# WQCG/blitzdg

Measured on AMD Instinct MI355X. Metric: element-DOF updates/sec (sw2d RHS + LSERK4 stage, N=4, 1M tris), higher is better.
Workload: dtype f64

## Files before the change

blitzdg_amd/csrc/hip/sw2d_affine_kernel.hpp:

```cpp
#pragma once
#include "sw2d_kernels.hpp"

namespace bdg_dev {

template <int N>
struct AffineOps {
    using E = Elem<N>;
    static constexpr int OFF_D = 0;
    static constexpr int OFF_LIFT = 2 * E::Np * E::Np;
    static constexpr int DOUBLES = OFF_LIFT + E::NFN * E::Np;
};

__device__ __forceinline__ double fast_rcp(double x) {
    double r = __builtin_amdgcn_rcp(x);
    r = fma(fma(-x, r, 1.0), r, r);
    r = fma(fma(-x, r, 1.0), r, r);
    return r;
}

__device__ __forceinline__ double fast_sqrt(double x) {
    x = fmax(x, 1e-290);
    const double y = __builtin_amdgcn_rsq(x);
    double g = x * y, h = 0.5 * y;
    const double r = fma(-h, g, 0.5);
    g = fma(g, r, g);
    h = fma(h, r, h);
    g = fma(fma(-g, g, x), h, g);
    return g;
}

template <typename T>
__device__ __forceinline__ T ld_row(const T* row, unsigned byteOff) {
    return *reinterpret_cast<const T*>(reinterpret_cast<const char*>(row) + byteOff);
}
template <typename T>
__device__ __forceinline__ void st_row(T* row, unsigned byteOff, T v) {
    *reinterpret_cast<T*>(reinterpret_cast<char*>(row) + byteOff) = v;
}

struct PhysParams {
    const double* sx;
    const double* sy;
    const double* fcor;
    const double* fmat;
    double fconst, cd, slope, dragSign;
    const double* H;
    const int* obc;
    const double* lam;
    const double* spongeField;
    double tide;
};

template <int N>
__device__ __forceinline__ unsigned link_node(unsigned code, int n) {
    using E = Elem<N>;
    const bool rev = (code & 4u) != 0;
    const unsigned f = code & 3u;
    const unsigned m0 = rev ? E::fmask(0, N - n) : E::fmask(0, n);
    const unsigned m1 = rev ? E::fmask(1, N - n) : E::fmask(1, n);
    const unsigned m2 = rev ? E::fmask(2, N - n) : E::fmask(2, n);
    return f == 0u ? m0 : (f == 1u ? m1 : m2);
}

constexpr int STAGE_VMAP = -1;

template <int N, int MODE, int PHYS = 0, bool TRACER = false, bool SPONGE = false, int KIND = STAGE_VMAP>
__global__ __launch_bounds__(256) void sw2d_stage_affine_kernel(const StageParams p, const PhysParams ph) {
    using E = Elem<N>;
    constexpr int Np = E::Np, Nfp = E::Nfp, NFN = E::NFN;
    constexpr bool kLinks = KIND != STAGE_VMAP;
    static_assert(!kLinks || (MODE == MODE_LSERK && PHYS == 0 && !TRACER && !SPONGE), "face links: three-field LSERK stages");
    constexpr bool kReadRes = MODE == MODE_LSERK && KIND != STAGE_FIRST;
    constexpr bool kWriteRes = KIND != STAGE_LAST;

    const unsigned nwg = gridDim.x, xcd = blockIdx.x % 8u, q8 = nwg / 8u, r8 = nwg % 8u;
    const unsigned tile = (xcd < r8 ? xcd * (q8 + 1u) : r8 * (q8 + 1u) + (xcd - r8) * q8) + blockIdx.x / 8u;
    const unsigned k = static_cast<unsigned>(p.kbegin) + tile * blockDim.x + threadIdx.x;
    if (k >= static_cast<unsigned>(p.kend)) return;
    const unsigned k8 = k * 8u, k4 = k * 4u;

    const long long ld = p.ld, plane = static_cast<long long>(Np) * ld;
    const double* __restrict__ ops = p.opsAffine;
    const double* __restrict__ qin = p.qin;

    int idx[kLinks ? 1 : NFN];
    unsigned lnk[kLinks ? 3 : 1];
    if constexpr (kLinks) {
        const unsigned* __restrict__ fl = reinterpret_cast<const unsigned*>(p.faceLink);
#pragma unroll
        for (int f = 0; f < 3; ++f) lnk[f] = ld_row(fl + f * ld, k4);
    } else {
#pragma unroll
        for (int j = 0; j < NFN; ++j) idx[j] = ld_row(p.vmapP + j * ld, k4);
    }
    double h[Np], hu[Np], hv[Np], hN[TRACER ? Np : 1];
#pragma unroll
    for (int n = 0; n < Np; ++n) {
        h[n] = ld_row(qin + n * ld, k8);
        hu[n] = ld_row(qin + plane + n * ld, k8);
        hv[n] = ld_row(qin + 2 * plane + n * ld, k8);
        if constexpr (TRACER) hN[n] = ld_row(qin + 3 * plane + n * ld, k8);
    }
    const double* __restrict__ ag = p.ageo;
    const double rx = ld_row(ag, k8), sx = ld_row(ag + ld, k8), ry = ld_row(ag + 2 * ld, k8), sy = ld_row(ag + 3 * ld, k8);
    double fnx[3], fny[3], fsc[3];
#pragma unroll
    for (int f = 0; f < 3; ++f) {
        fnx[f] = ld_row(ag + (4 + f) * ld, k8);
        fny[f] = ld_row(ag + (7 + f) * ld, k8);
        fsc[f] = ld_row(ag + (10 + f) * ld, k8);
    }
    double ssx[PHYS != 0 ? Np : 1], ssy[PHYS != 0 ? Np : 1], sfc[PHYS != 0 ? Np : 1];
    if constexpr (PHYS != 0) {
#pragma unroll
        for (int i = 0; i < Np; ++i) { ssx[i] = 0.0; ssy[i] = 0.0; sfc[i] = ph.fconst; }
        if (ph.sx) {
#pragma unroll
            for (int i = 0; i < Np; ++i) ssx[i] = ld_row(ph.sx + i * ld, k8);
        }
        if (ph.sy) {
#pragma unroll
            for (int i = 0; i < Np; ++i) ssy[i] = ld_row(ph.sy + i * ld, k8);
        }
        if (ph.fcor) {
#pragma unroll
            for (int i = 0; i < Np; ++i) sfc[i] = ld_row(ph.fcor + i * ld, k8);
        }
    }
    __builtin_amdgcn_sched_barrier(0);
    double hP[NFN], huP[NFN], hvP[NFN], hNP[TRACER ? NFN : 1];
    auto gatherFace = [&](int f) {
#pragma unroll
        for (int n = 0; n < Nfp; ++n) {
            const int j = f * Nfp + n;
            const unsigned o8 = static_cast<unsigned>(idx[j] < 0 ? -(idx[j] + 1) : idx[j]) * 8u;
            hP[j] = ld_row(qin, o8);
            huP[j] = ld_row(qin + plane, o8);
            hvP[j] = ld_row(qin + 2 * plane, o8);
            if constexpr (TRACER) hNP[j] = ld_row(qin + 3 * plane, o8);
        }
    };
    constexpr bool kLateFace = TRACER && MODE != MODE_LSERK;
    if constexpr (kLateFace) {
        gatherFace(0);
        gatherFace(1);
    } else if constexpr (kLinks) {
        const unsigned uld = static_cast<unsigned>(ld);
#pragma unroll
        for (int j = 0; j < NFN; ++j) {
            const int f = j / Nfp, n = j % Nfp;
            const unsigned code = lnk[f] >> FaceLink::FACE_SHIFT & 7u;
            const unsigned o8 = (link_node<N>(code, n) * uld + (lnk[f] & FaceLink::SLOT_MASK)) * 8u;
            hP[j] = ld_row(qin, o8);
            huP[j] = ld_row(qin + plane, o8);
            hvP[j] = ld_row(qin + 2 * plane, o8);
        }
    } else {
#pragma unroll
        for (int j = 0; j < NFN; ++j) {
            const unsigned o8 = static_cast<unsigned>(idx[j] < 0 ? -(idx[j] + 1) : idx[j]) * 8u;
            hP[j] = ld_row(qin, o8);
            huP[j] = ld_row(qin + plane, o8);
            hvP[j] = ld_row(qin + 2 * plane, o8);
            if constexpr (TRACER) hNP[j] = ld_row(qin + 3 * plane, o8);
        }
    }
    __builtin_amdgcn_sched_barrier(0);

    const double g = p.g, halfg = 0.5 * p.g;
    double R1[Np], R2[Np], R3[Np], R4[TRACER ? Np : 1];
#pragma unroll
    for (int i = 0; i < Np; ++i) R1[i] = R2[i] = R3[i] = 0.0;
    if constexpr (TRACER) {
#pragma unroll
        for (int i = 0; i < Np; ++i) R4[i] = 0.0;
    }
    if constexpr (PHYS != 0) {
#pragma unroll
        for (int m = 0; m < Np; ++m) {
            const double r = fast_rcp(h[m]);
            const double u = hu[m] * r, v = hv[m] * r;
            const double cdn = ph.cd * fast_sqrt(u * u + v * v);
            const double gh = ph.slope * g * h[m];
            R2[m] = fma(gh, ssx[m], fma(sfc[m], hv[m], -(cdn * u)));
            R3[m] = fma(gh, ssy[m], fma(ph.dragSign * cdn, v, -(sfc[m] * hu[m])));
        }
    }

#pragma unroll
    for (int f = 0; f < 3; ++f) {
        const double nxf = fnx[f], nyf = fny[f];
        double lam = 0.0;
        double uM[Nfp], vM[Nfp], uP[Nfp], vP[Nfp], hq[Nfp], huq[Nfp], hvq[Nfp];
#pragma unroll
        for (int n = 0; n < Nfp; ++n) {
            const int j = f * Nfp + n, m = E::fmask(f, n);
            const double rM = fast_rcp(h[m]);
            uM[n] = hu[m] * rM;
            vM[n] = hv[m] * rM;
            const double spdM = fast_sqrt(uM[n] * uM[n] + vM[n] * vM[n]) + fast_sqrt(g * h[m]);
            hq[n] = hP[j];
            huq[n] = huP[j];
            hvq[n] = hvP[j];
            bool wall;
            if constexpr (kLinks) wall = (lnk[f] & FaceLink::WALL) != 0u;
            else wall = idx[j] < 0;
            if (wall) {
                const double un = hu[m] * nxf + hv[m] * nyf;
                huq[n] = hu[m] - 2 * nxf * un;
                hvq[n] = hv[m] - 2 * nyf * un;
            }
            const double r = fast_rcp(hq[n]);
            uP[n] = huq[n] * r;
            vP[n] = hvq[n] * r;
            const double spdP = fast_sqrt(uP[n] * uP[n] + vP[n] * vP[n]) + fast_sqrt(g * hq[n]);
            lam = fmax(lam, fmax(spdM, spdP));
        }
        const double half_fs = 0.5 * fsc[f];
#pragma unroll
        for (int n = 0; n < Nfp; ++n) {
            const int j = f * Nfp + n, m = E::fmask(f, n);
            const double prM = halfg * h[m] * h[m], prP = halfg * hq[n] * hq[n];
            const double F2M = hu[m] * uM[n] + prM, G2M = hu[m] * vM[n], G3M = hv[m] * vM[n] + prM;
            const double F2P = huq[n] * uP[n] + prP, G2P = huq[n] * vP[n], G3P = hvq[n] * vP[n] + prP;
            const double dh = h[m] - hq[n], dhu = hu[m] - huq[n], dhv = hv[m] - hvq[n];
            const double s1 = half_fs * (dhu * nxf + dhv * nyf - lam * dh);
            const double s2 = half_fs * ((F2M - F2P) * nxf + (G2M - G2P) * nyf - lam * dhu);
            const double s3 = half_fs * ((G2M - G2P) * nxf + (G3M - G3P) * nyf - lam * dhv);
            double s4 = 0.0;
            if constexpr (TRACER)
                s4 = half_fs * ((hN[m] * uM[n] - hNP[j] * uP[n]) * nxf + (hN[m] * vM[n] - hNP[j] * vP[n]) * nyf -
                                lam * (hN[m] - hNP[j]));
#pragma unroll
            for (int i = 0; i < Np; ++i) {
                const double lj = ops[AffineOps<N>::OFF_LIFT + j * Np + i];
                R1[i] = fma(lj, s1, R1[i]);
                R2[i] = fma(lj, s2, R2[i]);
                R3[i] = fma(lj, s3, R3[i]);
                if constexpr (TRACER) R4[i] = fma(lj, s4, R4[i]);
            }
        }
        if constexpr (kLateFace) {
            if (f == 0) {
                gatherFace(2);
                __builtin_amdgcn_sched_barrier(0);
            }
        }
    }

    double old1[Np], old2[Np], old3[Np], old4[TRACER ? Np : 1];
    if constexpr (kReadRes) {
        const double* __restrict__ rs = p.res;
#pragma unroll
        for (int i = 0; i < Np; ++i) {
            old1[i] = ld_row(rs + i * ld, k8);
            old2[i] = ld_row(rs + plane + i * ld, k8);
            old3[i] = ld_row(rs + 2 * plane + i * ld, k8);
            if constexpr (TRACER) old4[i] = ld_row(rs + 3 * plane + i * ld, k8);
        }
    } else if constexpr (MODE == MODE_COMBINE) {
        const double* __restrict__ qb = p.qbase;
#pragma unroll
        for (int i = 0; i < Np; ++i) {
            old1[i] = ld_row(qb + i * ld, k8);
            old2[i] = ld_row(qb + plane + i * ld, k8);
            old3[i] = ld_row(qb + 2 * plane + i * ld, k8);
        }
    }
    __builtin_amdgcn_sched_barrier(0);

#pragma unroll
    for (int m = 0; m < Np; ++m) {
        const double r = fast_rcp(h[m] * p.one);
        const double u = hu[m] * r, v = hv[m] * r;
        const double pr = halfg * h[m] * h[m];
        const double F2 = hu[m] * u + pr, G2 = hu[m] * v, G3 = hv[m] * v + pr;
        const double a1 = -(rx * hu[m] + ry * hv[m]), b1 = -(sx * hu[m] + sy * hv[m]);
        const double a2 = -(rx * F2 + ry * G2), b2 = -(sx * F2 + sy * G2);
        const double a3 = -(rx * G2 + ry * G3), b3 = -(sx * G2 + sy * G3);
        double a4 = 0.0, b4 = 0.0;
        if constexpr (TRACER) {
            const double F4 = hN[m] * u, G4 = hN[m] * v;
            a4 = -(rx * F4 + ry * G4);
            b4 = -(sx * F4 + sy * G4);
        }
#pragma unroll
        for (int i = 0; i < Np; ++i) {
            const double dr = ops[AffineOps<N>::OFF_D + 2 * (m * Np + i)];
            R1[i] = fma(dr, a1, R1[i]);
            R2[i] = fma(dr, a2, R2[i]);
            R3[i] = fma(dr, a3, R3[i]);
            if constexpr (TRACER) R4[i] = fma(dr, a4, R4[i]);
        }
#pragma unroll
        for (int i = 0; i < Np; ++i) {
            const double ds = ops[AffineOps<N>::OFF_D + 2 * (m * Np + i) + 1];
            R1[i] = fma(ds, b1, R1[i]);
            R2[i] = fma(ds, b2, R2[i]);
            R3[i] = fma(ds, b3, R3[i]);
            if constexpr (TRACER) R4[i] = fma(ds, b4, R4[i]);
        }
    }

    if constexpr (PHYS == 2) {
        auto applyFilter = [&](double (&R)[Np]) {
            double T[Np];
#pragma unroll
            for (int i = 0; i < Np; ++i) T[i] = 0.0;
#pragma unroll
            for (int m = 0; m < Np; ++m)
#pragma unroll
                for (int i = 0; i < Np; ++i) T[i] = fma(ph.fmat[m * Np + i], R[m], T[i]);
#pragma unroll
            for (int i = 0; i < Np; ++i) R[i] = T[i];
        };
        applyFilter(R1);
        applyFilter(R2);
        applyFilter(R3);
        if constexpr (TRACER) applyFilter(R4);
    }

    if constexpr (TRACER && MODE == MODE_COMBINE) {
        const double* __restrict__ o4 = p.qbase + 3 * plane;
#pragma unroll
        for (int i = 0; i < Np; ++i) old4[i] = ld_row(o4 + i * ld, k8);
        __builtin_amdgcn_sched_barrier(0);
    }
    if constexpr (MODE == MODE_RHS) {
        double* __restrict__ o = p.rhs;
#pragma unroll
        for (int i = 0; i < Np; ++i) {
            st_row(o + i * ld, k8, R1[i]);
            st_row(o + plane + i * ld, k8, R2[i]);
            st_row(o + 2 * plane + i * ld, k8, R3[i]);
            if constexpr (TRACER) st_row(o + 3 * plane + i * ld, k8, R4[i]);
        }
    } else if constexpr (MODE == MODE_LSERK) {
        double* __restrict__ rs = p.res;
        double* __restrict__ o = p.qout;
        const double a = p.ca, b = p.cb, dt = p.cc;
#pragma unroll
        for (int i = 0; i < Np; ++i) {
            double n1, n2, n3;
            if constexpr (!kLinks) {
                n1 = a * old1[i] + dt * R1[i];
                n2 = a * old2[i] + dt * R2[i];
                n3 = a * old3[i] + dt * R3[i];
            } else if constexpr (kReadRes) {
                n1 = fma(dt, R1[i], a * old1[i]);
                n2 = fma(dt, R2[i], a * old2[i]);
                n3 = fma(dt, R3[i], a * old3[i]);
            } else {
                n1 = dt * R1[i];
                n2 = dt * R2[i];
                n3 = dt * R3[i];
            }
            if constexpr (kWriteRes) {
                st_row(rs + i * ld, k8, n1);
                st_row(rs + plane + i * ld, k8, n2);
                st_row(rs + 2 * plane + i * ld, k8, n3);
            }
            st_row(o + i * ld, k8, h[i] + b * n1);
            st_row(o + plane + i * ld, k8, hu[i] + b * n2);
            st_row(o + 2 * plane + i * ld, k8, hv[i] + b * n3);
            if constexpr (TRACER) {
                const double n4 = a * old4[i] + dt * R4[i];
                st_row(rs + 3 * plane + i * ld, k8, n4);
                st_row(o + 3 * plane + i * ld, k8, hN[i] + b * n4);
            }
        }
    } else {
        static_assert(!SPONGE || MODE == MODE_COMBINE, "the sponge follows a combine step");
        double* __restrict__ o = p.qout;
        const double a = p.ca, b = p.cb, c = p.cc;
        const double sg = p.sponge;
#pragma unroll
        for (int i = 0; i < Np; ++i) {
            const double v2 = a * old2[i] + b * hu[i] + c * R2[i], v3 = a * old3[i] + b * hv[i] + c * R3[i];
            st_row(o + i * ld, k8, a * old1[i] + b * h[i] + c * R1[i]);
            st_row(o + plane + i * ld, k8, SPONGE ? v2 / (1.0 + sg * v2 * v2) : v2);
            st_row(o + 2 * plane + i * ld, k8, SPONGE ? v3 / (1.0 + sg * v3 * v3) : v3);
        }
        if constexpr (TRACER) {
#pragma unroll
            for (int i = 0; i < Np; ++i) st_row(o + 3 * plane + i * ld, k8, a * old4[i] + b * hN[i] + c * R4[i]);
        }
    }
}

}

namespace bdg_dev {

template <int N, int MODE, int WAVES>
__global__ __launch_bounds__(256, WAVES) void sw2d_stage_affine_stream_kernel(const StageParams p) {
    using E = Elem<N>;
    constexpr int Np = E::Np, Nfp = E::Nfp;

    const unsigned nwg = gridDim.x, xcd = blockIdx.x % 8u, q8 = nwg / 8u, r8 = nwg % 8u;
    const unsigned tile = (xcd < r8 ? xcd * (q8 + 1u) : r8 * (q8 + 1u) + (xcd - r8) * q8) + blockIdx.x / 8u;
    const unsigned k = static_cast<unsigned>(p.kbegin) + tile * blockDim.x + threadIdx.x;
    if (k >= static_cast<unsigned>(p.kend)) return;
    const unsigned k8 = k * 8u, k4 = k * 4u;

    const long long ld = p.ld, plane = static_cast<long long>(Np) * ld;
    const double* __restrict__ ops = p.opsAffine;
    const double* __restrict__ qin = p.qin;
    const double* __restrict__ ag = p.ageo;
    const double g = p.g, halfg = 0.5 * p.g;

    double R1[Np], R2[Np], R3[Np];
#pragma unroll
    for (int i = 0; i < Np; ++i) R1[i] = R2[i] = R3[i] = 0.0;

    {
        const double rx = ld_row(ag, k8), sx = ld_row(ag + ld, k8), ry = ld_row(ag + 2 * ld, k8),
                     sy = ld_row(ag + 3 * ld, k8);
        constexpr int VCH = 5, NCH = (Np + VCH - 1) / VCH;
        double hc[2][VCH], huc[2][VCH], hvc[2][VCH];
#pragma unroll
        for (int t = 0; t < VCH; ++t)
            if (t < Np) {
                hc[0][t] = ld_row(qin + t * ld, k8);
                huc[0][t] = ld_row(qin + plane + t * ld, k8);
                hvc[0][t] = ld_row(qin + 2 * plane + t * ld, k8);
            }
#pragma unroll
        for (int c = 0; c < NCH; ++c) {
            const int cur = c & 1, nxt = cur ^ 1;
#pragma unroll
            for (int t = 0; t < VCH; ++t) {
                const int m = (c + 1) * VCH + t;
                if (m < Np) {
                    hc[nxt][t] = ld_row(qin + m * ld, k8);
                    huc[nxt][t] = ld_row(qin + plane + m * ld, k8);
                    hvc[nxt][t] = ld_row(qin + 2 * plane + m * ld, k8);
                }
            }
            __builtin_amdgcn_sched_barrier(0);
#pragma unroll
            for (int t = 0; t < VCH; ++t) {
                const int m = c * VCH + t;
                if (m < Np) {
                    const double h = hc[cur][t], hu = huc[cur][t], hv = hvc[cur][t];
                    const double r = fast_rcp(h);
                    const double u = hu * r, v = hv * r;
                    const double pr = halfg * h * h;
                    const double F2 = hu * u + pr, G2 = hu * v, G3 = hv * v + pr;
                    const double a1 = -(rx * hu + ry * hv), b1 = -(sx * hu + sy * hv);
                    const double a2 = -(rx * F2 + ry * G2), b2 = -(sx * F2 + sy * G2);
                    const double a3 = -(rx * G2 + ry * G3), b3 = -(sx * G2 + sy * G3);
#pragma unroll
                    for (int i = 0; i < Np; ++i) {
                        const double dr = ops[AffineOps<N>::OFF_D + 2 * (m * Np + i)];
                        R1[i] = fma(dr, a1, R1[i]);
                        R2[i] = fma(dr, a2, R2[i]);
                        R3[i] = fma(dr, a3, R3[i]);
                    }
#pragma unroll
                    for (int i = 0; i < Np; ++i) {
                        const double ds = ops[AffineOps<N>::OFF_D + 2 * (m * Np + i) + 1];
                        R1[i] = fma(ds, b1, R1[i]);
                        R2[i] = fma(ds, b2, R2[i]);
                        R3[i] = fma(ds, b3, R3[i]);
                    }
                }
            }
            __builtin_amdgcn_sched_barrier(0);
        }
    }
    __builtin_amdgcn_sched_barrier(0);

#pragma unroll
    for (int f = 0; f < 3; ++f) {
        const double nxf = ld_row(ag + (4 + f) * ld, k8), nyf = ld_row(ag + (7 + f) * ld, k8);
        const double half_fs = 0.5 * ld_row(ag + (10 + f) * ld, k8);
        int idx[Nfp];
        double hM[Nfp], huM[Nfp], hvM[Nfp], hq[Nfp], huq[Nfp], hvq[Nfp];
#pragma unroll
        for (int n = 0; n < Nfp; ++n) idx[n] = ld_row(p.vmapP + (f * Nfp + n) * ld, k4);
#pragma unroll
        for (int n = 0; n < Nfp; ++n) {
            const int m = E::fmask(f, n);
            hM[n] = ld_row(qin + m * ld, k8);
            huM[n] = ld_row(qin + plane + m * ld, k8);
            hvM[n] = ld_row(qin + 2 * plane + m * ld, k8);
        }
#pragma unroll
        for (int n = 0; n < Nfp; ++n) {
            const unsigned o8 = static_cast<unsigned>(idx[n] < 0 ? -(idx[n] + 1) : idx[n]) * 8u;
            hq[n] = ld_row(qin, o8);
            huq[n] = ld_row(qin + plane, o8);
            hvq[n] = ld_row(qin + 2 * plane, o8);
        }
        __builtin_amdgcn_sched_barrier(0);
        double lam = 0.0;
#pragma unroll
        for (int n = 0; n < Nfp; ++n) {
            if (idx[n] < 0) {
                const double un = huM[n] * nxf + hvM[n] * nyf;
                huq[n] = huM[n] - 2 * nxf * un;
                hvq[n] = hvM[n] - 2 * nyf * un;
            }
            const double rM = fast_rcp(hM[n]), rP = fast_rcp(hq[n]);
            const double uM = huM[n] * rM, vM = hvM[n] * rM, uP = huq[n] * rP, vP = hvq[n] * rP;
            const double spdM = fast_sqrt(uM * uM + vM * vM) + fast_sqrt(g * hM[n]);
            const double spdP = fast_sqrt(uP * uP + vP * vP) + fast_sqrt(g * hq[n]);
            lam = fmax(lam, fmax(spdM, spdP));
        }
#pragma unroll
        for (int n = 0; n < Nfp; ++n) {
            const int j = f * Nfp + n;
            const double rM = fast_rcp(hM[n] * p.one), rP = fast_rcp(hq[n] * p.one);
            const double uM = huM[n] * rM, vM = hvM[n] * rM, uP = huq[n] * rP, vP = hvq[n] * rP;
            const double prM = halfg * hM[n] * hM[n], prP = halfg * hq[n] * hq[n];
            const double F2M = huM[n] * uM + prM, G2M = huM[n] * vM, G3M = hvM[n] * vM + prM;
            const double F2P = huq[n] * uP + prP, G2P = huq[n] * vP, G3P = hvq[n] * vP + prP;
            const double dh = hM[n] - hq[n], dhu = huM[n] - huq[n], dhv = hvM[n] - hvq[n];
            const double s1 = half_fs * (dhu * nxf + dhv * nyf - lam * dh);
            const double s2 = half_fs * ((F2M - F2P) * nxf + (G2M - G2P) * nyf - lam * dhu);
            const double s3 = half_fs * ((G2M - G2P) * nxf + (G3M - G3P) * nyf - lam * dhv);
#pragma unroll
            for (int i = 0; i < Np; ++i) {
                const double lj = ops[AffineOps<N>::OFF_LIFT + j * Np + i];
                R1[i] = fma(lj, s1, R1[i]);
                R2[i] = fma(lj, s2, R2[i]);
                R3[i] = fma(lj, s3, R3[i]);
// ... 230 lines not shown
```

blitzdg_amd/csrc/hip/sw2d_device.hip:

```cpp
#include "../host/capi_internal.hpp"
#include "../host/element_order.hpp"
#include "../host/parallel_for.hpp"
#include "blitzdg/LSERK4.hpp"
#include "run_records.hpp"
#include "sw2d_launch.hpp"
#include "sw2d_launch_host.hpp"
#include "sw2d_drifter_kernel.hpp"
#include <algorithm>
#include <atomic>
#include <cmath>
#include <cstdlib>
#include <cstring>
#include <limits>
#include <queue>
#include <stdexcept>
#include <string>
#include <vector>

namespace bdg_dev {

const KernelTable* kernel_table_order1();
const KernelTable* kernel_table_order2();
const KernelTable* kernel_table_order3();
const KernelTable* kernel_table_order4();
// ... 686 lines not shown
                    img[o + 2] = F ? F[i * Np + m] : (i == m ? 1.0 : 0.0);
                }
            for (int j = 0; j < NFN; ++j)
                for (int i = 0; i < Np; ++i)
                    img[static_cast<size_t>(3) * Np * Np + static_cast<size_t>(j) * Np + i] = Lift[i * NFN + j];
            return img;
        };
        opsVd.upload(image(hostDr.data(), hostDs.data(), nullptr, hostLift.data()), bytes, "source ops upload");
        if (!hostFilter.empty())
            opsVdFiltered.upload(image(hostFDr.data(), hostFDs.data(), hostFilter.data(), hostFLift.data()), bytes,
                                 "filtered source ops upload");
    }

    void buildMfma2SourceOps() {
        if (opsMfma2Src.p) return;
        const int MT = kt->mfmaMT, KV = kt->mfmaKV, KF = kt->mfma2KF;
        auto image = [&](const double* Dr, const double* Ds, const double* Lift, const double* F) {
            const size_t tilesD = static_cast<size_t>(MT) * KV * 64, offF = static_cast<size_t>(kt->mfma2OpsDoubles);
            std::vector<double> img(offF + tilesD, 0.0);
            for (int r = 0; r < MT; ++r)
                for (int l = 0; l < 64; ++l) {
                    const int i = 16 * r + (l & 15);
                    if (i >= Np) continue;
                    for (int t = 0; t < KV; ++t) {
                        const int k = 4 * t + (l >> 4);
                        if (k >= Np) continue;
                        const size_t at = (static_cast<size_t>(r) * KV + t) * 64 + l;
                        img[at] = Dr[i * Np + k];
                        img[tilesD + at] = Ds[i * Np + k];
                        img[offF + at] = F ? F[i * Np + k] : (i == k ? 1.0 : 0.0);
                    }
                    for (int f = 0; f < 3; ++f)
                        for (int tf = 0; tf < KF; ++tf) {
                            const int n = 4 * tf + (l >> 4);
                            if (n < Nfp)
                                img[2 * tilesD + ((static_cast<size_t>(r) * 3 + f) * KF + tf) * 64 + l] = Lift[i * NFN + f * Nfp + n];
                        }
                }
            return img;
        };
        opsMfma2Src.upload(image(hostDr.data(), hostDs.data(), hostLift.data(), nullptr), bytes, "mfma2 source ops upload");
        if (!hostFilter.empty())
            opsMfma2SrcFiltered.upload(image(hostFDr.data(), hostFDs.data(), hostFLift.data(), hostFilter.data()), bytes,
                                       "filtered mfma2 source ops upload");
    }
    void buildFilterT() {
        if (filterT.p || hostFilter.empty()) return;
        std::vector<double> ft(static_cast<size_t>(Np) * Np);
        for (int m = 0; m < Np; ++m)
            for (int i = 0; i < Np; ++i) ft[static_cast<size_t>(m) * Np + i] = hostFilter[static_cast<size_t>(i) * Np + m];
        filterT.upload(ft, bytes, "filter upload");
    }

    void monitorReserve(long long steps, const char* fn) const { mon.reserve(steps, fn, "bdg_sw2d"); }
    void drifterReserve(long long steps, const char* fn) const { drf.reserve(steps, fn, "bdg_sw2d"); }
    long long lserkSteps(long long stages) const { return bdg_records::lserkSteps(stageCount, stages, blitzdg::LSERK4::numStages); }
    void monitorLaunch(double* rec, int capacity, int slot) {
        const double* Hm = mon.H.p ? mon.H.p : (hasH ? Hbuf.p : nullptr);
        mon.launch({qcur, Hm, ld, Np, nf, numOwned, g, timeNow}, rec, capacity, slot, bdg_dev::sw2d_monitor_finish_kernel,
                   "sw2d_monitor_finish_kernel launch", bdg_dev::MonRowGauges{mon.row.p}, stream);
    }
    void monitorSample() { monitorLaunch(mon.rec.p, mon.capacity, mon.count++); }
    void drifterLaunch(int mode, double dt, int slot) {
        drf.launch(bdg_dev::sw2d_drifter_kernel, "sw2d_drifter_kernel launch",
                   bdg_dev::TriDriftTables{drf.vert.p, drf.neigh.p, drf.vinvT.p, drf.jac.p}, qcur, ld, N, mode, dt, slot, stream);
    }
    void drifterAdvance(double dt, bool record = true) { drifterLaunch(bdg_dev::kDriftAdvance, dt, drf.takeSlot(record)); }
    void drifterResample() {
        if (drf.on) drifterLaunch(bdg_dev::kDriftSample, 0.0, -1);
    }
    void stepDone(double dt) {
        if (mon.on && ++mon.steps % mon.stride == 0) monitorSample();
        if (drf.on) {
            drf.t = timeNow;
            drifterAdvance(dt);
        }
    }
    void lserkStagesMonitored(int numStages) {
        for (int i = 0; i < numStages; ++i) {
            launchLserkStage();
            if (stageCount % blitzdg::LSERK4::numStages == 0) stepDone(dtStage);
        }
    }
    void lserkStagesExchangedMonitored(double dt, int numStages) {
        if (!mon.on) {
            launchLserkStagesExchanged(dt, numStages);
            return;
        }
        int left = numStages;
        while (left > 0) {
            const int toStep = blitzdg::LSERK4::numStages - static_cast<int>(stageCount % blitzdg::LSERK4::numStages);
            const long long stepsToDue = mon.stride - mon.steps % mon.stride;
            const long long want = toStep + (stepsToDue - 1) * blitzdg::LSERK4::numStages;
            const int piece = static_cast<int>(std::min<long long>(left, want));
            const long long done = lserkSteps(piece);
            launchLserkStagesExchanged(dt, piece);
            left -= piece;
            if (done > 0) {
                mon.steps += done - 1;
                stepDone(dt);
            }
        }
    }

    void reduceDt(double out[2]) {
        const int nblocks = (numOwned + 255) / 256;
        hipCheck(kt->dt(qcur, fscaleNodal, hasH ? Hbuf.p : nullptr, ld, numOwned, g, partials.p,
                        stream), "sw2d_dt_kernel");
        hipLaunchKernelGGL(bdg_dev::sw2d_reduce_kernel, dim3(1), dim3(256), 0, stream, partials.p, nblocks, red2.p);
        hipCheck(hipGetLastError(), "sw2d_reduce_kernel");
        hipCheck(hipMemcpyAsync(out, red2.p, 2 * sizeof(double), hipMemcpyDeviceToHost, stream), "D2H copy");
        hipCheck(hipStreamSynchronize(stream), "reduce sync");
    }
};

namespace {

bool geometryIsAffine(const bdg_sw2d_desc& d, int Np, int Nfp, int K) {
    const double tol = 1e-8;
    std::atomic<bool> ok{true};
    blitzdg::detail::parallelFor(K, [&](int k) {
        const double scale = std::fabs(d.rx[k]) + std::fabs(d.sx[k]) + std::fabs(d.ry[k]) + std::fabs(d.sy[k]);
        for (int n = 1; n < Np; ++n) {
            const size_t o = static_cast<size_t>(n) * K + k;
            if (std::fabs(d.rx[o] - d.rx[k]) > tol * scale || std::fabs(d.sx[o] - d.sx[k]) > tol * scale ||
                std::fabs(d.ry[o] - d.ry[k]) > tol * scale || std::fabs(d.sy[o] - d.sy[k]) > tol * scale)
                ok = false;
        }
        for (int f = 0; f < 3; ++f) {
            const size_t o0 = static_cast<size_t>(f) * Nfp * K + k;
            for (int n = 1; n < Nfp; ++n) {
                const size_t o = o0 + static_cast<size_t>(n) * K;
                if (std::fabs(d.nx[o] - d.nx[o0]) > tol || std::fabs(d.ny[o] - d.ny[o0]) > tol ||
                    std::fabs(d.Fscale[o] - d.Fscale[o0]) > tol * std::fabs(d.Fscale[o0]))
                    ok = false;
            }
        }
    });
    return ok;
}

std::vector<double> matmulHost(const double* A, const double* B, int n, int c) {
    std::vector<double> C(static_cast<size_t>(n) * c, 0.0);
    for (int i = 0; i < n; ++i)
        for (int j = 0; j < c; ++j) {
            double s = 0.0;
            for (int k = 0; k < n; ++k) s += A[i * n + k] * B[k * c + j];
            C[static_cast<size_t>(i) * c + j] = s;
        }
    return C;
}

std::vector<double> affineOpsImage(const double* Dr, const double* Ds, const double* Lift, int Np, int NFN) {
    std::vector<double> img(static_cast<size_t>(2) * Np * Np + static_cast<size_t>(NFN) * Np);
    for (int m = 0; m < Np; ++m)
        for (int i = 0; i < Np; ++i) {
            img[2 * (static_cast<size_t>(m) * Np + i)] = Dr[i * Np + m];
            img[2 * (static_cast<size_t>(m) * Np + i) + 1] = Ds[i * Np + m];
        }
    for (int j = 0; j < NFN; ++j)
        for (int i = 0; i < Np; ++i) img[static_cast<size_t>(2) * Np * Np + static_cast<size_t>(j) * Np + i] = Lift[i * NFN + j];
    return img;
}

bdg_sw2d* createSolver(const bdg_sw2d_desc& d) {
    if (d.order < 1 || d.order > BDG_SW2D_MAX_ORDER)
        throw arg_error("bdg_sw2d_create: order must be 1.." + std::to_string(BDG_SW2D_MAX_ORDER) +
                        " for the register-resident kernels");
    if (d.num_elements < 1) throw arg_error("bdg_sw2d_create: num_elements must be >= 1");
    if (!d.Dr || !d.Ds || !d.Lift || !d.rx || !d.sx || !d.ry || !d.sy || !d.nx || !d.ny || !d.Fscale || !d.vmapP)
        throw arg_error("bdg_sw2d_create: a required table pointer is NULL");
    if (d.num_wall < 0 || (d.num_wall > 0 && !d.mapW)) throw arg_error("bdg_sw2d_create: bad wall-node list");

    const bdg_dev::KernelTable* kt = bdg_dev::kernel_table(d.order);
    if (!kt) throw arg_error("bdg_sw2d_create: no kernels compiled for this order");

    int ndev = 0;
    if (hipGetDeviceCount(&ndev) != hipSuccess || ndev < 1)
        throw hip_error("bdg_sw2d_create: no HIP device available (the sw2d path has no CPU fallback)");
    if (d.device < 0 || d.device >= ndev) throw arg_error("bdg_sw2d_create: device ordinal out of range");

    auto s = std::unique_ptr<bdg_sw2d>(new bdg_sw2d());
    s->kt = kt;
    s->N = d.order; s->Np = kt->Np; s->Nfp = kt->Nfp; s->NFN = 3 * kt->Nfp; s->K = d.num_elements;
    s->device = d.device;
    s->g = d.g;
    if (d.num_fields != 0 && d.num_fields != 3 && d.num_fields != 4)
        throw arg_error("bdg_sw2d_create: num_fields must be 3 or 4");
    s->nf = d.num_fields == 4 ? 4 : 3;
    s->variantD = s->nf == 4 || d.sources != 0;
    s->ld = (static_cast<long long>(s->K) + 63) / 64 * 64;
    s->numInterior = s->numOwned = s->K;
    const int Np = s->Np, Nfp = s->Nfp, NFN = s->NFN, K = s->K;
    const long long ld = s->ld;
    if (static_cast<long long>(Np) * ld * 8 > 4294967295LL)
        throw arg_error("bdg_sw2d_create: Np*K exceeds 2^29 nodes (32-bit byte offsets within a field): partition the "
                        "mesh over more devices");

    const size_t nFaceNodes = static_cast<size_t>(NFN) * K;
    if (d.vmapM)
        for (int k = 0; k < K; ++k)
            for (int f = 0; f < 3; ++f)
                for (int n = 0; n < Nfp; ++n)
                    if (d.vmapM[(static_cast<size_t>(k) * 3 + f) * Nfp + n] != kt->fmask(f, n) + Np * k)
                        throw arg_error("bdg_sw2d_create: vmapM does not follow the warp&blend face-node ordering "
                                        "(Fmask) these kernels are specialised for");
    const long long totalNodes = static_cast<long long>(Np) * K;
    for (size_t i = 0; i < nFaceNodes; ++i)
        if (d.vmapP[i] < 0 || d.vmapP[i] >= totalNodes) throw arg_error("bdg_sw2d_create: vmapP entry out of range");
    for (int i = 0; i < d.num_wall; ++i)
        if (d.mapW[i] < 0 || static_cast<size_t>(d.mapW[i]) >= nFaceNodes)
            throw arg_error("bdg_sw2d_create: wall-node index out of range");

    namespace eo = blitzdg::element_order;
    const bool reorder = (d.flags & BDG_SW2D_REORDER) != 0 ||
                         (!(d.flags & BDG_SW2D_KEEP_ORDER) && eo::renumberingWanted(d.vmapP, K, Np, Nfp, d.order));
    if (reorder) s->permHost = eo::renumbering(d.vmapP, K, Np, Nfp, eo::patchSetting());
    s->affine = !(d.flags & BDG_SW2D_NODAL_GEOMETRY) && geometryIsAffine(d, Np, Nfp, K);
    s->nodalMfma = !s->affine && !(env::nodalVector() && kt->ldsDoubles != 0);

    s->use();
    hipCheck(hipStreamCreateWithFlags(&s->stream, hipStreamNonBlocking), "hipStreamCreate");

    const size_t plane3 = static_cast<size_t>(s->nf) * s->planeSize();
    s->qA.alloc(plane3, s->bytes);
    s->qB.alloc(plane3, s->bytes);
    s->res.alloc(plane3, s->bytes);
    s->aux.alloc(plane3, s->bytes);
    const size_t fplane = static_cast<size_t>(NFN) * ld;
    if (!s->affine) {
        s->geo.alloc(4 * s->planeSize(), s->bytes);
        s->fgeo.alloc(3 * fplane, s->bytes);
        s->ops.alloc(kt->ldsDoubles, s->bytes);
    } else {
        s->fgeo.alloc(fplane, s->bytes);
    }
    s->fscaleNodal = s->affine ? s->fgeo.p : s->fgeo.p + 2 * fplane;
    s->vmapP.alloc(static_cast<size_t>(NFN) * ld, s->bytes);
    s->stage.alloc(static_cast<size_t>(std::max(Np, NFN)) * K, s->bytes);
    s->istage.alloc(static_cast<size_t>(NFN) * K, s->bytes);
    s->partials.alloc(2 * static_cast<size_t>((K + 255) / 256), s->bytes);
    s->red2.alloc(2, s->bytes);
    if (!s->permHost.empty()) s->perm.upload(s->permHost, s->bytes, "perm upload");
    for (auto* b : {&s->qA, &s->qB, &s->res, &s->aux, &s->geo, &s->fgeo})
        if (b->p) hipCheck(hipMemsetAsync(b->p, 0, b->n * sizeof(double), s->stream), "hipMemset");
    hipCheck(hipMemsetAsync(s->vmapP.p, 0, s->vmapP.n * sizeof(int), s->stream), "hipMemset");
    s->qcur = s->qA.p;
    s->qalt = s->qB.p;

    s->hasFilter = d.Filter != nullptr;
    if (!s->affine && kt->ldsDoubles > 0) {
        std::vector<double> img(kt->ldsDoubles, 0.0);
        for (int i = 0; i < Np * Np; ++i) {
            img[2 * i] = d.Dr[i];
            img[2 * i + 1] = d.Ds[i];
        }
        std::copy(d.Lift, d.Lift + static_cast<size_t>(Np) * NFN, img.begin() + 2 * Np * Np);
        if (d.Filter) std::copy(d.Filter, d.Filter + static_cast<size_t>(Np) * Np, img.begin() + 2 * Np * Np + Np * NFN);
        hipCheck(hipMemcpyAsync(s->ops.p, img.data(), img.size() * sizeof(double), hipMemcpyHostToDevice, s->stream),
                 "ops upload");
        hipCheck(hipStreamSynchronize(s->stream), "ops sync");
    }

    if (!s->affine) {
        const size_t pl = s->planeSize();
        s->uploadRows(d.rx, s->geo.p, Np);
        s->uploadRows(d.sx, s->geo.p + pl, Np);
        s->uploadRows(d.ry, s->geo.p + 2 * pl, Np);
        s->uploadRows(d.sy, s->geo.p + 3 * pl, Np);
        s->uploadRows(d.nx, s->fgeo.p, NFN);
        s->uploadRows(d.ny, s->fgeo.p + fplane, NFN);
    }
    s->uploadRows(d.Fscale, s->fscaleNodal, NFN);

    s->affineVariant = s->N <= 4 ? bdg_dev::AffineVariant::Unrolled : bdg_dev::AffineVariant::Mfma3;
    if (const char* e = env::affineVariantPin()) {
        const int v = std::atoi(e);
        if (v >= 0 && v <= 9) {
            s->affineVariant = static_cast<bdg_dev::AffineVariant>(v);
            s->variantForced = true;
        }
    }
    s->hostDr.assign(d.Dr, d.Dr + static_cast<size_t>(Np) * Np);
    s->hostDs.assign(d.Ds, d.Ds + static_cast<size_t>(Np) * Np);
    s->hostLift.assign(d.Lift, d.Lift + static_cast<size_t>(Np) * NFN);
    if (d.Filter) {
        s->hostFilter.assign(d.Filter, d.Filter + static_cast<size_t>(Np) * Np);
        s->hostFDr = matmulHost(d.Filter, d.Dr, Np, Np);
        s->hostFDs = matmulHost(d.Filter, d.Ds, Np, Np);
        s->hostFLift = matmulHost(d.Filter, d.Lift, Np, NFN);
    }
    auto mfmaImage = [&](const double* Dr, const double* Ds, const double* Lift) {
        const int MT = kt->mfmaMT, KV = kt->mfmaKV, KS = kt->mfmaKS;
        std::vector<double> img(static_cast<size_t>(kt->mfmaOpsDoubles), 0.0);
        auto fill = [&](size_t off, const double* A, int cols, int KT) {
            for (int r = 0; r < MT; ++r)
                for (int t = 0; t < KT; ++t)
                    for (int l = 0; l < 64; ++l) {
                        const int i = 16 * r + (l & 15), k = 4 * t + (l >> 4);
                        if (i < Np && k < cols) img[off + (static_cast<size_t>(r) * KT + t) * 64 + l] = A[i * cols + k];
                    }
        };
        fill(0, Dr, Np, KV);
        fill(static_cast<size_t>(MT) * KV * 64, Ds, Np, KV);
        fill(static_cast<size_t>(2) * MT * KV * 64, Lift, NFN, KS);
        return img;
    };
// ... 1054 lines not shown
```

Before: 43.36 billion.

## Stream affine operator matrices through double-buffered scalar load windows

For the N=4 face-link LSERK kernel, the Lift and Dr/Ds operator entries are now fetched with explicit s_load_dwordx16 instructions into SGPR windows. Two 64-byte blocks make up a window, the next window is requested while the current one is consumed, and each window is gated by an explicit lgkmcnt wait. This is meant to hide scalar-load latency that the compiler schedule leaves exposed. The Dr and Ds loops are interleaved to match the stream order, scalar parameters are pinned into SGPRs, and the host op image is padded to whole 8-double blocks. The hand-placed waits and sched barriers constrain the compiler's scheduling, and the SGPR pressure may rise. Microbenchmark and asm scan tools are added as well.

```diff
diff --git a/blitzdg_amd/csrc/hip/sw2d_affine_kernel.hpp b/blitzdg_amd/csrc/hip/sw2d_affine_kernel.hpp
--- a/blitzdg_amd/csrc/hip/sw2d_affine_kernel.hpp
+++ b/blitzdg_amd/csrc/hip/sw2d_affine_kernel.hpp
@@ -9,6 +9,22 @@
     static constexpr int OFF_D = 0;
     static constexpr int OFF_LIFT = 2 * E::Np * E::Np;
     static constexpr int DOUBLES = OFF_LIFT + E::NFN * E::Np;
+    static constexpr int BLOCK = 8;
+    static constexpr int PADDED = (DOUBLES + BLOCK - 1) / BLOCK * BLOCK;
+    static_assert(PADDED % BLOCK == 0 && PADDED >= DOUBLES && PADDED - DOUBLES < BLOCK, "whole blocks, nothing read past the allocation");
+};
+
+template <int N>
+struct OpStream {
+    using O = AffineOps<N>;
+    static constexpr int B = O::BLOCK, W = 2;
+    static constexpr int LIFT_FIRST = O::OFF_LIFT / B;
+    static constexpr int LIFT_BLOCKS = O::PADDED / B - LIFT_FIRST;
+    static constexpr int D_BLOCKS = (O::OFF_LIFT + B - 1) / B;
+    static constexpr int BLOCKS = LIFT_BLOCKS + D_BLOCKS, WINDOWS = (BLOCKS + W - 1) / W;
+    static constexpr int seq(int e) { return e >= O::OFF_LIFT ? e / B - LIFT_FIRST : LIFT_BLOCKS + e / B; }
+    static constexpr int block(int sb) { return sb < LIFT_BLOCKS ? LIFT_FIRST + sb : sb - LIFT_BLOCKS; }
+    static constexpr bool opens(int e) { return seq(e) % W == 0 && (e % B == 0 || e == O::OFF_LIFT); }
 };
 
 __device__ __forceinline__ double fast_rcp(double x) {
@@ -83,6 +99,31 @@
     const double* __restrict__ ops = p.opsAffine;
     const double* __restrict__ qin = p.qin;
 
+    constexpr bool kStream = kLinks && N == 4;
+    using OS = OpStream<N>;
+    typedef double OpBlock __attribute__((ext_vector_type(8)));
+    static_assert(OS::B == 8 && OS::W == 2, "one s_load_dwordx16 per block, two blocks named by the wait");
+    OpBlock win[2][OS::W];
+    auto requestWindow = [&](int w) {
+#pragma unroll
+        for (int t = 0; t < OS::W; ++t) {
+            const int sb = w * OS::W + t < OS::BLOCKS ? w * OS::W + t : OS::BLOCKS - 1;
+            const unsigned byteOff = OS::block(sb) * OS::B * 8;
+            asm volatile("s_load_dwordx16 %0, %1, %2" : "=s"(win[w & 1][t]) : "s"(ops), "s"(byteOff));
+        }
+    };
+    auto op = [&](int e) -> double {
+        const int sb = OS::seq(e), w = sb / OS::W;
+        if (OS::opens(e)) {
+            __builtin_amdgcn_sched_barrier(0);
+            asm volatile("s_waitcnt lgkmcnt(0)" : "+s"(win[w & 1][0]), "+s"(win[w & 1][1]));
+            if (w + 1 < OS::WINDOWS) requestWindow(w + 1);
+            __builtin_amdgcn_sched_barrier(0);
+        }
+        return win[w & 1][sb % OS::W][e % OS::B];
+    };
+
+    if constexpr (kStream) requestWindow(0);
     int idx[kLinks ? 1 : NFN];
     unsigned lnk[kLinks ? 3 : 1];
     if constexpr (kLinks) {
@@ -127,6 +168,8 @@
             for (int i = 0; i < Np; ++i) sfc[i] = ld_row(ph.fcor + i * ld, k8);
         }
     }
+    double sG = p.g, sA = p.ca, sB = p.cb, sC = p.cc, sOne = p.one;
+    if constexpr (kStream) asm("" : "+s"(sG), "+s"(sA), "+s"(sB), "+s"(sC), "+s"(sOne));
     __builtin_amdgcn_sched_barrier(0);
     double hP[NFN], huP[NFN], hvP[NFN], hNP[TRACER ? NFN : 1];
     auto gatherFace = [&](int f) {
@@ -167,7 +210,7 @@
     }
     __builtin_amdgcn_sched_barrier(0);
 
-    const double g = p.g, halfg = 0.5 * p.g;
+    const double g = sG, halfg = 0.5 * sG;
     double R1[Np], R2[Np], R3[Np], R4[TRACER ? Np : 1];
 #pragma unroll
     for (int i = 0; i < Np; ++i) R1[i] = R2[i] = R3[i] = 0.0;
@@ -233,7 +276,9 @@
                                 lam * (hN[m] - hNP[j]));
 #pragma unroll
             for (int i = 0; i < Np; ++i) {
-                const double lj = ops[AffineOps<N>::OFF_LIFT + j * Np + i];
+                double lj;
+                if constexpr (kStream) lj = op(AffineOps<N>::OFF_LIFT + j * Np + i);
+                else lj = ops[AffineOps<N>::OFF_LIFT + j * Np + i];
                 R1[i] = fma(lj, s1, R1[i]);
                 R2[i] = fma(lj, s2, R2[i]);
                 R3[i] = fma(lj, s3, R3[i]);
@@ -271,7 +316,7 @@
 
 #pragma unroll
     for (int m = 0; m < Np; ++m) {
-        const double r = fast_rcp(h[m] * p.one);
+        const double r = fast_rcp(h[m] * sOne);
         const double u = hu[m] * r, v = hv[m] * r;
         const double pr = halfg * h[m] * h[m];
         const double F2 = hu[m] * u + pr, G2 = hu[m] * v, G3 = hv[m] * v + pr;
@@ -284,21 +329,35 @@
             a4 = -(rx * F4 + ry * G4);
             b4 = -(sx * F4 + sy * G4);
         }
-#pragma unroll
-        for (int i = 0; i < Np; ++i) {
-            const double dr = ops[AffineOps<N>::OFF_D + 2 * (m * Np + i)];
-            R1[i] = fma(dr, a1, R1[i]);
-            R2[i] = fma(dr, a2, R2[i]);
-            R3[i] = fma(dr, a3, R3[i]);
-            if constexpr (TRACER) R4[i] = fma(dr, a4, R4[i]);
-        }
-#pragma unroll
-        for (int i = 0; i < Np; ++i) {
-            const double ds = ops[AffineOps<N>::OFF_D + 2 * (m * Np + i) + 1];
-            R1[i] = fma(ds, b1, R1[i]);
-            R2[i] = fma(ds, b2, R2[i]);
-            R3[i] = fma(ds, b3, R3[i]);
-            if constexpr (TRACER) R4[i] = fma(ds, b4, R4[i]);
+        if constexpr (kStream) {
+#pragma unroll
+            for (int i = 0; i < Np; ++i) {
+                const double dr = op(AffineOps<N>::OFF_D + 2 * (m * Np + i));
+                R1[i] = fma(dr, a1, R1[i]);
+                R2[i] = fma(dr, a2, R2[i]);
+                R3[i] = fma(dr, a3, R3[i]);
+                const double ds = op(AffineOps<N>::OFF_D + 2 * (m * Np + i) + 1);
+                R1[i] = fma(ds, b1, R1[i]);
+                R2[i] = fma(ds, b2, R2[i]);
+                R3[i] = fma(ds, b3, R3[i]);
+            }
+        } else {
+#pragma unroll
+            for (int i = 0; i < Np; ++i) {
+                const double dr = ops[AffineOps<N>::OFF_D + 2 * (m * Np + i)];
+                R1[i] = fma(dr, a1, R1[i]);
+                R2[i] = fma(dr, a2, R2[i]);
+                R3[i] = fma(dr, a3, R3[i]);
+                if constexpr (TRACER) R4[i] = fma(dr, a4, R4[i]);
+            }
+#pragma unroll
+            for (int i = 0; i < Np; ++i) {
+                const double ds = ops[AffineOps<N>::OFF_D + 2 * (m * Np + i) + 1];
+                R1[i] = fma(ds, b1, R1[i]);
+                R2[i] = fma(ds, b2, R2[i]);
+                R3[i] = fma(ds, b3, R3[i]);
+                if constexpr (TRACER) R4[i] = fma(ds, b4, R4[i]);
+            }
         }
     }
 
@@ -338,7 +397,7 @@
     } else if constexpr (MODE == MODE_LSERK) {
         double* __restrict__ rs = p.res;
         double* __restrict__ o = p.qout;
-        const double a = p.ca, b = p.cb, dt = p.cc;
+        const double a = sA, b = sB, dt = sC;
 #pragma unroll
         for (int i = 0; i < Np; ++i) {
             double n1, n2, n3;
@@ -372,7 +431,7 @@
     } else {
         static_assert(!SPONGE || MODE == MODE_COMBINE, "the sponge follows a combine step");
         double* __restrict__ o = p.qout;
-        const double a = p.ca, b = p.cb, c = p.cc;
+        const double a = sA, b = sB, c = sC;
         const double sg = p.sponge;
 #pragma unroll
         for (int i = 0; i < Np; ++i) {
diff --git a/blitzdg_amd/csrc/hip/sw2d_device.hip b/blitzdg_amd/csrc/hip/sw2d_device.hip
--- a/blitzdg_amd/csrc/hip/sw2d_device.hip
+++ b/blitzdg_amd/csrc/hip/sw2d_device.hip
@@ -862,7 +862,8 @@
 }
 
 std::vector<double> affineOpsImage(const double* Dr, const double* Ds, const double* Lift, int Np, int NFN) {
-    std::vector<double> img(static_cast<size_t>(2) * Np * Np + static_cast<size_t>(NFN) * Np);
+    const size_t doubles = static_cast<size_t>(2) * Np * Np + static_cast<size_t>(NFN) * Np;
+    std::vector<double> img((doubles + 7) / 8 * 8, 0.0);
     for (int m = 0; m < Np; ++m)
         for (int i = 0; i < Np; ++i) {
             img[2 * (static_cast<size_t>(m) * Np + i)] = Dr[i * Np + m];
diff --git a/profiles/microbench/scalar_load_latency.hip b/profiles/microbench/scalar_load_latency.hip
--- /dev/null
+++ b/profiles/microbench/scalar_load_latency.hip
@@ -0,0 +1,147 @@
+#include <hip/hip_runtime.h>
+#include <algorithm>
+#include <cstdio>
+#include <vector>
+
+typedef unsigned v16u __attribute__((ext_vector_type(16)));
+
+constexpr int BLOCK_BYTES = 64;
+constexpr int NBLOCKS = 88;
+constexpr int PASSES = 16;
+
+#define FMA8                                  \
+    "v_fma_f64 %[x0], %[x0], %[m], %[c]\n\t"  \
+    "v_fma_f64 %[x1], %[x1], %[m], %[c]\n\t"  \
+    "v_fma_f64 %[x2], %[x2], %[m], %[c]\n\t"  \
+    "v_fma_f64 %[x3], %[x3], %[m], %[c]\n\t"  \
+    "v_fma_f64 %[x4], %[x4], %[m], %[c]\n\t"  \
+    "v_fma_f64 %[x5], %[x5], %[m], %[c]\n\t"  \
+    "v_fma_f64 %[x6], %[x6], %[m], %[c]\n\t"  \
+    "v_fma_f64 %[x7], %[x7], %[m], %[c]\n\t"
+#define FMA0 ""
+#define FMA24 FMA8 FMA8 FMA8
+#define FMA48 FMA24 FMA24
+#define FMA96 FMA48 FMA48
+#define LOAD0 ""
+#define LOAD1 "s_load_dwordx16 %[a], %[base], %[o0]\n\t"
+#define LOAD2 LOAD1 "s_load_dwordx16 %[b], %[base], %[o1]\n\t"
+#define LOAD4 LOAD2 "s_load_dwordx16 %[c4], %[base], %[o2]\n\t" "s_load_dwordx16 %[d], %[base], %[o3]\n\t"
+
+struct Acc {
+    double x[8];
+};
+
+#define PROBE(NAME, K, LOADS, FMAS)                                                                                          \
+    __global__ __launch_bounds__(64) void NAME(const char* image, float* warm, float* cold, double* sink, double m, double c) { \
+        extern __shared__ char occupancy_pad[];                                                                              \
+        Acc r;                                                                                                               \
+        for (int i = 0; i < 8; ++i) r.x[i] = threadIdx.x + i;                                                                \
+        unsigned long long warmTicks = 0, coldTicks = 0;                                                                     \
+        unsigned keep = 0, groups = 0;                                                                                       \
+        for (int pass = 0; pass < PASSES; ++pass) {                                                                          \
+            for (int blk = 0; blk < NBLOCKS; blk += (K ? K : 1)) {                                                           \
+                const unsigned o0 = blk * BLOCK_BYTES, o1 = o0 + BLOCK_BYTES, o2 = o0 + 2 * BLOCK_BYTES,                     \
+                               o3 = o0 + 3 * BLOCK_BYTES;                                                                    \
+                unsigned long long t0, t1;                                                                                   \
+                v16u a = {}, b = {}, c4 = {}, d = {};                                                                        \
+                asm volatile("s_memtime %[t0]\n\ts_waitcnt lgkmcnt(0)\n\t" LOADS FMAS                                        \
+                             "s_waitcnt lgkmcnt(0)\n\ts_memtime %[t1]\n\ts_waitcnt lgkmcnt(0)\n\t"                           \
+                             : [t0] "=&s"(t0), [t1] "=&s"(t1), [a] "+s"(a), [b] "+s"(b), [c4] "+s"(c4), [d] "+s"(d),         \
+                               [x0] "+v"(r.x[0]), [x1] "+v"(r.x[1]), [x2] "+v"(r.x[2]), [x3] "+v"(r.x[3]),                   \
+                               [x4] "+v"(r.x[4]), [x5] "+v"(r.x[5]), [x6] "+v"(r.x[6]), [x7] "+v"(r.x[7])                    \
+                             : [base] "s"(image), [o0] "s"(o0), [o1] "s"(o1), [o2] "s"(o2), [o3] "s"(o3), [m] "v"(m),        \
+                               [c] "v"(c)                                                                                    \
+                             : "memory");                                                                                    \
+                keep ^= a[0] ^ b[3] ^ c4[7] ^ d[15];                                                                         \
+                if (pass == 0) coldTicks += t1 - t0;                                                                         \
+                else warmTicks += t1 - t0;                                                                                   \
+                if (pass == 0) ++groups;                                                                                     \
+            }                                                                                                                \
+        }                                                                                                                    \
+        double s = keep;                                                                                                     \
+        for (int i = 0; i < 8; ++i) s += r.x[i];                                                                             \
+        sink[blockIdx.x * 64 + threadIdx.x] = s;                                                                             \
+        if (threadIdx.x == 0) {                                                                                              \
+            warm[blockIdx.x] = static_cast<float>(warmTicks) / static_cast<float>(groups * (PASSES - 1));                    \
+            cold[blockIdx.x] = static_cast<float>(coldTicks) / static_cast<float>(groups);                                   \
+        }                                                                                                                    \
+    }
+
+#define PROBES_FOR(F)                          \
+    PROBE(probe_k0_f##F, 0, LOAD0, FMA##F)     \
+    PROBE(probe_k1_f##F, 1, LOAD1, FMA##F)     \
+    PROBE(probe_k2_f##F, 2, LOAD2, FMA##F)     \
+    PROBE(probe_k4_f##F, 4, LOAD4, FMA##F)
+PROBES_FOR(0)
+PROBES_FOR(24)
+PROBES_FOR(48)
+PROBES_FOR(96)
+
+__global__ void clock_kernel(unsigned long long* out) {
+    const unsigned long long r0 = __builtin_amdgcn_s_memrealtime(), t0 = __builtin_amdgcn_s_memtime();
+    unsigned long long r1 = r0;
+    while (r1 - r0 < 20000000ull) r1 = __builtin_amdgcn_s_memrealtime();
+    out[0] = __builtin_amdgcn_s_memtime() - t0;
+    out[1] = r1 - r0;
+}
+
+using Kernel = void (*)(const char*, float*, float*, double*, double, double);
+struct Probe {
+    int k, f;
+    Kernel fn;
+};
+
+static float median(std::vector<float> v) {
+    std::sort(v.begin(), v.end());
+    return v[v.size() / 2];
+}
+
+int main() {
+    hipDeviceProp_t prop;
+    if (hipGetDeviceProperties(&prop, 0) != hipSuccess) return 1;
+    const int nwg = prop.multiProcessorCount * 4;
+    const size_t lds = 40 * 1024;
+    std::vector<double> img(NBLOCKS * BLOCK_BYTES / 8);
+    for (size_t i = 0; i < img.size(); ++i) img[i] = 1.0 / (1.0 + i);
+    char* dimg;
+    float *dwarm, *dcold;
+    double* dsink;
+    unsigned long long* dclk;
+    if (hipMalloc(&dimg, img.size() * 8) != hipSuccess) return 1;
+    if (hipMalloc(&dwarm, nwg * 4) != hipSuccess || hipMalloc(&dcold, nwg * 4) != hipSuccess ||
+        hipMalloc(&dsink, nwg * 64 * 8) != hipSuccess || hipMalloc(&dclk, 16) != hipSuccess) return 1;
+    if (hipMemcpy(dimg, img.data(), img.size() * 8, hipMemcpyHostToDevice) != hipSuccess) return 1;
+
+#define ROW(F) {0, F, probe_k0_f##F}, {1, F, probe_k1_f##F}, {2, F, probe_k2_f##F}, {4, F, probe_k4_f##F}
+    const Probe probes[] = {ROW(0), ROW(24), ROW(48), ROW(96)};
+    const int np = sizeof(probes) / sizeof(probes[0]);
+    std::vector<float> warm(np), cold(np), hw(nwg), hc(nwg);
+    for (int rep = 0; rep < 2; ++rep)
+        for (int i = 0; i < np; ++i) {
+            hipLaunchKernelGGL(probes[i].fn, dim3(nwg), dim3(64), lds, 0, dimg, dwarm, dcold, dsink, 1.0000001, 1e-9);
+            if (hipDeviceSynchronize() != hipSuccess) { std::printf("probe %d failed\n", i); return 1; }
+            if (hipMemcpy(hw.data(), dwarm, nwg * 4, hipMemcpyDeviceToHost) != hipSuccess ||
+                hipMemcpy(hc.data(), dcold, nwg * 4, hipMemcpyDeviceToHost) != hipSuccess) return 1;
+            warm[i] = median(hw);
+            cold[i] = median(hc);
+        }
+    hipLaunchKernelGGL(clock_kernel, dim3(1), dim3(1), 0, 0, dclk);
+    unsigned long long clk[2];
+    if (hipMemcpy(clk, dclk, 16, hipMemcpyDeviceToHost) != hipSuccess) return 1;
+
+    std::printf("%s, %d CUs, %d workgroups of one wave, image %d B in %d-byte blocks, %d passes\n", prop.gcnArchName,
+                prop.multiProcessorCount, nwg, NBLOCKS * BLOCK_BYTES, BLOCK_BYTES, PASSES);
+    std::printf("shader clock while spinning: %.0f MHz (s_memtime ticks per s_memrealtime tick x 100 MHz)\n",
+                100.0 * static_cast<double>(clk[0]) / static_cast<double>(clk[1]));
+    std::printf("ticks between the stamps, median over workgroups (warm passes | cold pass):\n");
+    std::printf("  %-8s %-8s %12s %12s %14s %14s\n", "loads K", "FMAs F", "T warm", "T cold", "T - T(0,F) warm", "T - T(0,F) cold");
+    for (int i = 0; i < np; ++i) {
+        const int base = i / 4 * 4;
+        std::printf("  %-8d %-8d %12.1f %12.1f %14.1f %14.1f\n", probes[i].k, probes[i].f, warm[i], cold[i],
+                    warm[i] - warm[base], cold[i] - cold[base]);
+    }
+    std::printf("round trip of K loads issued together, warm: K=1 %.1f, K=2 %.1f, K=4 %.1f ticks\n", warm[1] - warm[0],
+                warm[2] - warm[0], warm[3] - warm[0]);
+    std::printf("one fp64 FMA: %.2f ticks (from F = 96 against F = 0 without loads)\n", (warm[12] - warm[0]) / 96.0);
+    return 0;
+}
diff --git a/profiles/scalar_wait_scan.py b/profiles/scalar_wait_scan.py
--- /dev/null
+++ b/profiles/scalar_wait_scan.py
@@ -0,0 +1,78 @@
+#!/usr/bin/env python3
+import re
+import sys
+
+RT1, RT_NEXT, VALU_TICKS = 48.3, 16.0, 4.5
+
+KERNEL = re.compile(r"^(_ZN7bdg_dev\w+):")
+INSTR = re.compile(r"^\s+([a-z_0-9]+)\b(.*)$")
+
+
+def kernels(text):
+    out, name = {}, None
+    for line in text.splitlines():
+        m = KERNEL.match(line)
+        if m:
+            name = m.group(1)
+            out[name] = []
+            continue
+        if name is None:
+            continue
+        for mark, pseudo in (("; sched_barrier", "sched_barrier"), (";;#ASMSTART", "asmstart"), (";;#ASMEND", "asmend")):
+            if line.lstrip().startswith(mark):
+                out[name].append((pseudo, ""))
+        m = INSTR.match(line)
+        if not m or line.lstrip().startswith((".", ";")):
+            continue
+        out[name].append((m.group(1), m.group(2)))
+        if m.group(1) == "s_endpgm":
+            name = None
+    return out
+
+
+def scan(instrs):
+    waits, started, pending, fmas, valu, other = [], False, 0, 0, 0, 0
+    for op, args in instrs:
+        if op in ("asmstart", "asmend"):
+            continue
+        if op == "sched_barrier":
+            started = True
+        elif op.startswith("s_load") or op.startswith("s_buffer_load"):
+            pending += 1
+            fmas = valu = other = 0
+        elif op == "s_waitcnt" and "lgkmcnt(0)" in args:
+            if pending and started:
+                cover = valu * VALU_TICKS + other
+                waits.append(dict(loads=pending, fmas=fmas, valu=valu, other=other,
+                                  exposed=max(0.0, RT1 + (pending - 1) * RT_NEXT - cover)))
+            pending = 0
+        elif op.startswith("v_"):
+            valu += 1
+            fmas += op.startswith(("v_fma_f64", "v_fmac_f64"))
+        else:
+            other += 1
+    return waits
+
+
+def summary(instrs):
+    count = lambda pred: sum(1 for op, _ in instrs if pred(op))
+    return dict(valu=count(lambda o: o.startswith("v_")), s_load=count(lambda o: o.startswith("s_load")),
+                s_load_x16=count(lambda o: o == "s_load_dwordx16"), v_lshl_add_u64=count(lambda o: o == "v_lshl_add_u64"),
+                v_readlane=count(lambda o: o == "v_readlane_b32"), v_writelane=count(lambda o: o == "v_writelane_b32"),
+                v_accvgpr=count(lambda o: o.startswith("v_accvgpr")))
+
+
+if __name__ == "__main__":
+    for name, instrs in kernels(open(sys.argv[1]).read().replace("\\\n", "")).items():
+        waits = scan(instrs)
+        print(name)
+        print("  ", summary(instrs))
+        if not waits:
+            continue
+        print(f"   {len(waits)} scalar waits behind the first batch; fp64 FMAs between the youngest load and the wait: "
+              f"min {min(w['fmas'] for w in waits)}, "
+              f"sorted {sorted(w['fmas'] for w in waits)}")
+        print(f"   estimated ticks no instruction covers: {sum(w['exposed'] for w in waits):.0f}")
+        if "-v" in sys.argv:
+            for w in waits:
+                print("     ", w)
```

Result: no change. 43.77 billion (median of 6 runs) (+0.9%).
